# emdgroup/baybe

Measured on AMD Instinct MI355X. Metric: acquisition candidates scored/sec (1e6 discrete grid, n_train=512, qLogEI), higher is better.
Workload: dtype f64; 1 GPU; 1000000 x 20 discrete grid per GPU, n_train=512, Matern-5/2 ARD, qLogEI S=512, fixed-theta, top-8 to host; global_rows=1000000, parallelism=row-shard x1, collective=none

## Files before the change

baybe_amd/csrc/bbh_coop.h:

```cpp
#pragma once
#define BBH_CANDREG 1
#include "bbh_fused.h"

#define BBH_COOP_ROUNDS 8
#define BBH_COOP_KV_TILE (2 * 4 * 256)
#ifndef BBH_COOP_WAVES
#define BBH_COOP_WAVES 2
#endif
#ifndef BBH_COOP_PAIRS
#define BBH_COOP_PAIRS 4
#endif
#ifndef BBH_COOP_ABLATE_BARRIER
#define BBH_COOP_ABLATE_BARRIER 0
#endif
#ifndef BBH_COOP_ABLATE_MEM
#define BBH_COOP_ABLATE_MEM 0
#endif
#ifndef BBH_COOP_ABLATE_PRO
#define BBH_COOP_ABLATE_PRO 0
#endif
#ifndef BBH_COOP_ABLATE_LOADS
#define BBH_COOP_ABLATE_LOADS 0
#endif
#ifndef BBH_COOP_ABLATE_CHAIN
#define BBH_COOP_ABLATE_CHAIN 0
#endif
#ifndef BBH_COOP_ABLATE_KV
#define BBH_COOP_ABLATE_KV 0
#endif

typedef double d2 __attribute__((ext_vector_type(2)));
template <int IMM>
__device__ __forceinline__ void coop_gload2(d2& dst, const double* sbase, unsigned voff) {
  static_assert(IMM >= 0 && IMM + 16 <= 4096, "13-bit signed immediate offset");
  asm volatile("global_load_dwordx4 %0, %1, %2 offset:%3" : "=v"(dst) : "v"(voff), "s"(sbase), "n"(IMM));
}
template <int N>
__device__ __forceinline__ void coop_vmwait2(d2& slot) {
  asm volatile("s_waitcnt vmcnt(%1)" : "+v"(slot) : "n"(N));
}
template <int IMM>
__device__ __forceinline__ void coop_gload(double& dst, const double* sbase, unsigned voff) {
  static_assert(IMM >= 0 && IMM < 4096, "13-bit signed immediate offset");
  asm volatile("global_load_dwordx2 %0, %1, %2 offset:%3" : "=v"(dst) : "v"(voff), "s"(sbase), "n"(IMM));
}
template <int N>
__device__ __forceinline__ void coop_vmwait(double& slot) {
  asm volatile("s_waitcnt vmcnt(%1)" : "+v"(slot) : "n"(N));
}

struct CoopArgs {
  FusedArgs f;
  const double* rstream;
  int64_t frags;
  int g0;
  const double* na = nullptr;
};

__host__ __device__ constexpr int coop_frags_before(int G) { return 16 * (G * BBH_COOP_ROUNDS - (G * (G - 1)) / 2); }

template <int G, int KD, int KVF, bool PRODUCE, int NT, bool OPEN = false>
__device__ __forceinline__ void coop_group(const WaveCtx (&c)[NT], const double* rs, const double* tfn, const bbh_lds_double* kv_cur,
                                           bbh_lds_double* kv_mine_next, const bbh_lds_double* alpha_next, int tbn, int cw,
                                           d4 (&acc)[NT][BBH_COOP_ROUNDS], d2 (&ring)[BBH_COOP_PAIRS], double (&accm)[NT],
                                           const bbh_lds_double* na_next = (const bbh_lds_double*)nullptr) {
  constexpr bool SEED = (KVF & 8) != 0;
  constexpr int NP = BBH_COOP_PAIRS;
  constexpr int CNT = BBH_COOP_ROUNDS - G;
  constexpr int FULL = CNT - 1;
  constexpr int TOT = 16 * CNT;
  constexpr int REM = OPEN ? (1 << 20) : coop_frags_before(BBH_COOP_ROUNDS) - coop_frags_before(G + 1);
  constexpr int HOSTS = 12 * FULL;
  constexpr int STEPS = NT * BBH_KV_STEPS;
  const unsigned lane8 = (unsigned)c[0].l * 8u, lane16 = (unsigned)c[0].l * 16u;
  double tfv[KD];
  d4 dsa[NT], dsb[NT];
  KvState<BBH_KV_NU> P;
  double kv[NT][4], kvx[NT][4], kvn[NT][4], alv[4], nav[4];
  if constexpr (PRODUCE && SEED) {
#pragma unroll
    for (int r = 0; r < 4; r++) nav[r] = na_next[4 * r];
  }
  if constexpr (PRODUCE) {
    static_for<0, KD>([&](auto kc) __attribute__((always_inline)) {
      constexpr int k = decltype(kc)::value;
      coop_gload<(k % 8) * 512>(tfv[k], tfn + (k / 8) * 512, lane8);
    });
  }
#pragma unroll
  for (int t = 0; t < NT; t++)
#pragma unroll
    for (int r = 0; r < 4; r++) kv[t][r] = kv_cur[t * BBH_COOP_KV_TILE + r * 64];
  __builtin_amdgcn_sched_barrier(0);
  static_for<0, 4>([&](auto ic) __attribute__((always_inline)) {
    constexpr int i = decltype(ic)::value;
    if constexpr (i < 3) {
#pragma unroll
      for (int t = 0; t < NT; t++)
#pragma unroll
        for (int r = 0; r < 4; r++) kvx[t][r] = kv_cur[t * BBH_COOP_KV_TILE + (i + 1) * 256 + r * 64];
    } else if constexpr (PRODUCE) {
#pragma unroll
      for (int r = 0; r < 4; r++) alv[r] = alpha_next[4 * r];
    }
    static_for<0, 4>([&](auto rc) __attribute__((always_inline)) {
      constexpr int r = decltype(rc)::value;
      static_for<0, CNT>([&](auto sc) __attribute__((always_inline)) {
        constexpr int s = decltype(sc)::value;
        constexpr int f = (i * 4 + r) * CNT + s;
        constexpr int pr = f / 2;
        if constexpr (f % 2 == 0 && !BBH_COOP_ABLATE_LOADS) {
          constexpr int BEHIND = ((TOT + REM) / 2 - 1 - pr) < (NP - 1) ? ((TOT + REM) / 2 - 1 - pr) : (NP - 1);
          coop_vmwait2<BEHIND + ((PRODUCE && pr < NP) ? KD : 0)>(ring[pr % NP]);
        }
#if BBH_COOP_ABLATE_CHAIN
        static_for<0, NT>([&](auto tc_) __attribute__((always_inline)) {
          constexpr int t = decltype(tc_)::value;
          if constexpr (s == 0) {
            if (cw >= i) acc[t][f % 8] = mfma_f64(kv[t][r], ring[pr % NP][f % 2], acc[t][f % 8]);
          } else {
            acc[t][f % 8] = mfma_f64(kv[t][r], ring[pr % NP][f % 2], acc[t][f % 8]);
          }
        });
#else
        static_for<0, NT>([&](auto tc_) __attribute__((always_inline)) {
          constexpr int t = decltype(tc_)::value;
          if constexpr (s == 0) {
            if (cw >= i) acc[t][G] = mfma_f64(kv[t][r], ring[pr % NP][f % 2], acc[t][G]);
          } else {
            acc[t][G + s] = mfma_f64(kv[t][r], ring[pr % NP][f % 2], acc[t][G + s]);
          }
        });
#endif
        if constexpr (f % 2 == 1 && 2 * (pr + NP) < TOT + REM && !BBH_COOP_ABLATE_LOADS) {
          constexpr int np = pr + NP;
          coop_gload2<(np % 4) * 1024>(ring[pr % NP], BBH_COOP_ABLATE_MEM ? rs : rs + (np / 4) * 512, lane16);
        }
        if constexpr (PRODUCE && i >= 1 && s >= 1 && !BBH_COOP_ABLATE_KV) {
          constexpr int m = ((i - 1) * 4 + r) * FULL + (s - 1);
          static_for<(m * STEPS) / HOSTS, ((m + 1) * STEPS) / HOSTS>([&](auto st) __attribute__((always_inline)) {
            constexpr int tile = decltype(st)::value / BBH_KV_STEPS, micro = decltype(st)::value % BBH_KV_STEPS;
            kv_micro<KVF, BBH_KV_NU, micro>(P, c[tile], tbn, 0, dsa[tile], dsb[tile], kvn[tile]);
          });
        }
        __builtin_amdgcn_sched_barrier(0);
      });
      if constexpr (PRODUCE && i == 0 && r == 3) {
        coop_vmwait<NP>(tfv[KD - 1]);
        __builtin_amdgcn_sched_barrier(0);
        if constexpr (!BBH_COOP_ABLATE_KV) {
          static_for<0, NT>([&](auto tc_) __attribute__((always_inline)) {
            constexpr int t = decltype(tc_)::value;
            if constexpr (SEED) {
              const d4 seed = {nav[0] + c[t].nbn, nav[1] + c[t].nbn, nav[2] + c[t].nbn, nav[3] + c[t].nbn};
              kvp_dist_seeded<KD>(c[t], tfv, seed, dsa[t], dsb[t]);
            } else {
              kvp_dist<KD>(c[t], tfv, dsa[t], dsb[t]);
            }
          });
        }
      }
    });
    if constexpr (i < 3) {
#pragma unroll
      for (int t = 0; t < NT; t++)
#pragma unroll
        for (int r = 0; r < 4; r++) kv[t][r] = kvx[t][r];
    }
  });
  if constexpr (PRODUCE) {
#pragma unroll
    for (int t = 0; t < NT; t++)
#pragma unroll
      for (int r = 0; r < 4; r++) {
        if constexpr (BBH_COOP_ABLATE_KV) kvn[t][r] = tfv[r];
        kv_mine_next[t * BBH_COOP_KV_TILE + r * 64] = kvn[t][r];
        accm[t] = fma(kvn[t][r], alv[r], accm[t]);
      }
  }
}

template <int KD, int KVF, int NT, int GMIN = 0>
__global__ __launch_bounds__(256, (GMIN >= 6 ? 5 : GMIN >= 4 ? 4 : BBH_COOP_WAVES)) void bbh_coop_posterior_kernel(const CoopArgs ca) {
  const FusedArgs& a = ca.f;
  extern __shared__ __attribute__((aligned(16))) double s_mem[];
  constexpr bool SEED = (KVF & 8) != 0;
  static_assert(!SEED || (KVF & 6) == 0, "the seeded stream carries the Matern-5/2 constant");
  const int l = threadIdx.x & 63, w = __builtin_amdgcn_readfirstlane(threadIdx.x >> 6);
  const int cnd = l & 15, q = l >> 4;
  double* s_alpha = s_mem;
  double* s_na = s_alpha + 16 * a.nb;
  double* s_kv = s_na + (SEED ? 16 * a.nb : 0);
  double* s_red = s_kv + NT * BBH_COOP_KV_TILE;
  const int64_t tile0 = (int64_t)blockIdx.x * (16 * NT);

  WaveCtx c[NT];
  int tcs[NT];
  int xcol[KD];
  double xval[NT][KD], xscl[KD], xofs[KD];
  const double* xr[NT];
  double tfv0[KD];
  kvp_load<KD>(a.trainfrag + l, w, tfv0);
  double na0[4];
  if constexpr (SEED) {
#pragma unroll
    for (int r = 0; r < 4; r++) na0[r] = ca.na[16 * w + 4 * r + q];
  }
#pragma unroll
  for (int t = 0; t < NT; t++) {
    const int64_t row = (tile0 + 16 * t + cnd < a.N) ? tile0 + 16 * t + cnd : a.N - 1;
    xr[t] = a.X + row * a.ldx;
  }
  if (a.numcol_identity) {
#pragma unroll
    for (int k = 0; k < KD; k++) xcol[k] = (4 * k + q < a.dn) ? 4 * k + q : a.dn - 1;
  } else {
#pragma unroll
    for (int k = 0; k < KD; k++) xcol[k] = a.numcol[(4 * k + q < a.dn) ? 4 * k + q : a.dn - 1];
  }
#pragma unroll
  for (int k = 0; k < KD; k++) {
    const int dimc = (4 * k + q < a.dn) ? 4 * k + q : a.dn - 1;
#pragma unroll
    for (int t = 0; t < NT; t++) xval[t][k] = xr[t][xcol[k]];
    xscl[k] = a.scl[dimc];
    xofs[k] = a.ofs[dimc];
  }
  if (!(BBH_COOP_ABLATE_PRO & 1))
    for (int s = threadIdx.x; s < 16 * a.nb; s += 256) s_alpha[s] = a.meanB[(int64_t)s * 16];
  if constexpr (SEED)
    for (int s = threadIdx.x; s < 16 * a.nb; s += 256) s_na[s] = ca.na[s];
#pragma unroll
  for (int t = 0; t < NT; t++) {
    double nbsum = 0.0;
#pragma unroll
    for (int k = 0; k < KD; k++) {
      const int dim = 4 * k + q;
      double v = 0.0;
      if (dim < a.dn) {
        v = (BBH_COOP_ABLATE_PRO & 2) ? 0.01 * (double)(dim + cnd) : fma(xval[t][k], xscl[k], xofs[k]);
        if constexpr (SEED) v *= BBH_SQRT5;
        nbsum = fma(v, v, nbsum);
      }
      c[t].cf[k] = v;
    }
    nbsum += __shfl_xor(nbsum, 16, 64);
    nbsum += __shfl_xor(nbsum, 32, 64);
    if constexpr (!SEED) {
#pragma unroll
      for (int k = 0; k < KD; k++) {
        if (4 * k + q == a.dn) c[t].cf[k] = 1.0;
        if (4 * k + q == a.dn + 1) c[t].cf[k] = nbsum;
      }
    }
    c[t].nbn = nbsum;
    int tc = 0;
    if constexpr ((KVF & 1) != 0) {
      if (a.task_col >= 0) {
        tc = (int)xr[t][a.task_col];
        tc = tc < 0 ? 0 : (tc >= a.T ? a.T - 1 : tc);
      }
    }
    tcs[t] = tc;
    c[t].tf = a.trainfrag + l;
    c[t].candl = nullptr;
    c[t].mb = nullptr;
    c[t].tbl = a.tasktbl;
    c[t].taskext = a.taskext;
    c[t].kvc = nullptr;
    c[t].kvl = (bbh_lds_double*)nullptr;
    c[t].nl = 0;
    c[t].ncache = 0;
    c[t].al = (const bbh_lds_double*)nullptr;
    c[t].kd = KD;
    c[t].kind = a.kind;
    c[t].T = a.T;
    c[t].tc = tc;
    c[t].q = q;
    c[t].l = l;
    c[t].dn = a.dn;
  }

  bbh_lds_double* kvb = (bbh_lds_double*)(s_kv + l);
  const bbh_lds_double* alq = (const bbh_lds_double*)(s_alpha + q);
  const bbh_lds_double* naq = (const bbh_lds_double*)(s_na + q);
  const int g0 = ca.g0;
  double accm[NT];
  d4 acc[NT][BBH_COOP_ROUNDS];
#pragma unroll
  for (int t = 0; t < NT; t++) {
    accm[t] = 0.0;
#pragma unroll
    for (int s = 0; s < BBH_COOP_ROUNDS; s++) acc[t][s] = (d4){0.0, 0.0, 0.0, 0.0};
  }
  const double* rs = ca.rstream + (int64_t)w * ca.frags * 64;
  d2 ring[BBH_COOP_PAIRS];
  static_for<0, BBH_COOP_PAIRS>([&](auto ic) __attribute__((always_inline)) {
    constexpr int i = decltype(ic)::value;
    coop_gload2<(i % 4) * 1024>(ring[i], rs + (i / 4) * 512, (unsigned)l * 16u);
  });
  {
    double tfv[KD], kv0[NT][4];
    if constexpr (BBH_COOP_ABLATE_PRO & 4) {
      for (int t = 0; t < NT; t++)
        for (int r = 0; r < 4; r++) kv0[t][r] = 0.5 + 0.001 * (double)(l + r);
    } else {
#pragma unroll
      for (int k = 0; k < KD; k++) tfv[k] = tfv0[k];
#pragma unroll
      for (int t = 0; t < NT; t++) {
        d4 dsa, dsb;
        if constexpr (SEED) {
          const d4 seed = {na0[0] + c[t].nbn, na0[1] + c[t].nbn, na0[2] + c[t].nbn, na0[3] + c[t].nbn};
          kvp_dist_seeded<KD>(c[t], tfv, seed, dsa, dsb);
        } else {
          kvp_dist<KD>(c[t], tfv, dsa, dsb);
        }
        kv_all<KVF>(c[t], w, dsa, dsb, kv0[t]);
      }
    }
    __syncthreads();
#pragma unroll
    for (int t = 0; t < NT; t++)
#pragma unroll
      for (int r = 0; r < 4; r++) {
        kvb[t * BBH_COOP_KV_TILE + ((g0 & 1) * 4 + w) * 256 + r * 64] = kv0[t][r];
        accm[t] = fma(kv0[t][r], alq[16 * w + 4 * r], accm[t]);
      }
  }
  __syncthreads();

  static_for<GMIN, BBH_COOP_ROUNDS>([&](auto gc) __attribute__((always_inline)) {
    constexpr int G = decltype(gc)::value;
    if (G >= g0) {
      const int cw = (G & 1) ? 3 - w : w;
      const int tbn = 4 * (G + 1 - g0) + w;
      constexpr bool PRODUCE = G + 1 < BBH_COOP_ROUNDS;
      coop_group<G, KD, KVF, PRODUCE, NT>(c, rs, a.trainfrag + (int64_t)tbn * KD * 64, kvb + (G & 1) * 4 * 256,
                                          kvb + (((G + 1) & 1) * 4 + w) * 256, alq + 16 * tbn, tbn, cw, acc, ring, accm, naq + 16 * tbn);
      rs += (int64_t)16 * (BBH_COOP_ROUNDS - G) * 64;
#if !BBH_COOP_ABLATE_BARRIER
      if constexpr (PRODUCE) __syncthreads();
#endif
    }
  });

  if constexpr (BBH_COOP_ABLATE_PRO & 8) {
    double keep = 0.0;
#pragma unroll
    for (int t = 0; t < NT; t++) {
      keep += accm[t];
#pragma unroll
      for (int s = 0; s < BBH_COOP_ROUNDS; s++) keep += (acc[t][s][0] + acc[t][s][1]) + (acc[t][s][2] + acc[t][s][3]);
    }
    if (l == 0 && w == 0) a.var[tile0] = keep;
    return;
  }
#pragma unroll
  for (int t = 0; t < NT; t++) {
    double ss[4] = {0.0, 0.0, 0.0, 0.0};
#pragma unroll
    for (int s = 0; s < BBH_COOP_ROUNDS; s++)
#pragma unroll
      for (int r = 0; r < 4; r++) ss[r] = fma(acc[t][s][r], acc[t][s][r], ss[r]);
#pragma unroll
    for (int r = 0; r < 4; r++) {
      double v = ss[r];
      v += __shfl_xor(v, 1, 64);
      v += __shfl_xor(v, 2, 64);
      v += __shfl_xor(v, 4, 64);
      v += __shfl_xor(v, 8, 64);
      ss[r] = v;
    }
    double mp = accm[t];
    mp += __shfl_xor(mp, 16, 64);
    mp += __shfl_xor(mp, 32, 64);
    double* red_v = s_red + t * 128;
    double* red_m = red_v + 64;
    if (cnd == 0) {
#pragma unroll
      for (int r = 0; r < 4; r++) red_v[w * 16 + q + 4 * r] = ss[r];
    }
    if (q == 0) red_m[w * 16 + cnd] = mp;
  }
  __syncthreads();
  if (threadIdx.x < 16 * NT) {
    const int m = threadIdx.x & 15, t = threadIdx.x >> 4;
    const int64_t gi = tile0 + 16 * t + m;
    const double* red_v = s_red + t * 128;
    const double* red_m = red_v + 64;
    const double sv = (red_v[m] + red_v[16 + m]) + (red_v[32 + m] + red_v[48 + m]);
    const double sm = (red_m[m] + red_m[16 + m]) + (red_m[32 + m] + red_m[48 + m]);
    double pv = a.prior_scale, mc = a.mean_const;
    if constexpr ((KVF & 1) != 0) {
      int tcm = __shfl(tcs[0], m, 64);
      if constexpr (NT > 1) {
        const int tcm1 = __shfl(tcs[NT - 1], m, 64);
        tcm = t ? tcm1 : tcm;
      }
      pv = a.tasktbl[tcm * a.T + tcm];
      if (a.taskmean) mc = a.taskmean[tcm];
    }
    if (gi < a.N) {
      if (a.mean) a.mean[gi] = a.ybar + a.ysd * (mc + sm);
      if (a.var) a.var[gi] = a.ysd * a.ysd * (pv - sv);
    }
  }
}

bool bbh_coop_launch(int kd, int kind, bool has_tbl, dim3 grid, size_t lds, hipStream_t s, const CoopArgs& a, bool small_ok);
bool bbh_coop_launch_a(int kd, int kind, bool has_tbl, dim3 grid, size_t lds, hipStream_t s, const CoopArgs& a);
bool bbh_coop_launch_b(int kd, int kind, bool has_tbl, dim3 grid, size_t lds, hipStream_t s, const CoopArgs& a);
bool bbh_coop_launch_small(int kd, int kind, bool has_tbl, dim3 grid, size_t lds, hipStream_t s, const CoopArgs& a);
bool bbh_coop_seed_launch(int kds, bool has_tbl, dim3 grid, size_t lds, hipStream_t s, const CoopArgs& a, bool small_ok);
bool bbh_coop_seed_launch_small(int kds, bool has_tbl, dim3 grid, size_t lds, hipStream_t s, const CoopArgs& a);

#define BBH_COOP_DISPATCH_KD(KDV, NTV)                                                                                        \
  if (kd == KDV) {                                                                                                       \
    const bool m52 = kind == BBH_KERNEL_MATERN52, rbf = kind == BBH_KERNEL_RBF, plain = kind == BBH_KERNEL_MATERN32 && !has_tbl; \
    if (!m52 && !rbf && !plain) return false;                                                                            \
    if (grid.x == 0) return true;                                                                                        \
    if (rbf && has_tbl)                                                       \
      hipLaunchKernelGGL((bbh_coop_posterior_kernel<KDV, 3, NTV>), grid, dim3(256), lds, s, a);                               \
    else if (rbf)                                                                                                        \
      hipLaunchKernelGGL((bbh_coop_posterior_kernel<KDV, 2, NTV>), grid, dim3(256), lds, s, a);                               \
    else if (kind == BBH_KERNEL_MATERN32)                                                                                \
      hipLaunchKernelGGL((bbh_coop_posterior_kernel<KDV, 4, NTV>), grid, dim3(256), lds, s, a);                               \
    else if (has_tbl)                                                                                                    \
      hipLaunchKernelGGL((bbh_coop_posterior_kernel<KDV, 1, NTV>), grid, dim3(256), lds, s, a);                               \
    else                                                                                                                 \
      hipLaunchKernelGGL((bbh_coop_posterior_kernel<KDV, 0, NTV>), grid, dim3(256), lds, s, a);                               \
    return true;                                                                                                         \
  }
```

baybe_amd/csrc/bbh_fused.h:

```cpp
#pragma once
#include <math.h>
#include <string.h>

#include <type_traits>

#include "bbh_common.h"

#define BBH_MAX_PASS 64
#ifndef BBH_W32_REMAINDERS
#define BBH_W32_REMAINDERS 0
#endif

__device__ __forceinline__ double bbh_kfun_p(int kind, double r2) {
  if (kind == BBH_KERNEL_RBF) return exp(-0.5 * r2);
  const double r = sqrt(r2);
  if (kind == BBH_KERNEL_MATERN52) return (1.0 + BBH_SQRT5 * r + (5.0 / 3.0) * r2) * exp(-BBH_SQRT5 * r);
  if (kind == BBH_KERNEL_MATERN32) return (1.0 + BBH_SQRT3 * r) * exp(-BBH_SQRT3 * r);
  return exp(-r);
}

struct FusedArgs {
  const double* X;
  int64_t N, ldx;
  const double* trainfrag;
  const double* rfrag;
  const double* meanB;
  const double* scl;
  const double* ofs;
  const int* numcol;
  const double* tasktbl;
  const double* taskmean;
  const int* taskext;
  double* mean;
  double* var;
  double* cross;
  const int64_t* pass_off;
  const int* pass_w;
  int npass;
  int kind, dn, kd, nb, nb_ext, task_col, T, p, with_var;
  double ybar, ysd, mean_const, prior_scale;
  const double* qz;
  int qS;
  double q_best_f, q_sign;
  const uint8_t* q_alive;
  double* q_scores;
  double* kvcache;
  int* slab_flags;
  int nslab, nxcc;
  int ncache;
  int64_t nblk;
  int nl;
  int has_tbl;
  int mean_valu;
  int numcol_identity;
};

typedef __attribute__((address_space(3))) double bbh_lds_double;

struct WaveCtx {
  const double* tf;
  const double* candl;
  const double* mb;
  const double* tbl;
  const int* taskext;
  double* kvc;
  bbh_lds_double* kvl;
  int nl, ncache;
  const bbh_lds_double* al;
  int kd, kind, T, tc, q, l, dn;
  double nbn;
  double cf[16];
};

#ifndef BBH_CANDREG
#define BBH_CANDREG 0
#endif
#ifndef BBH_DIST_ASM
#define BBH_DIST_ASM 0
#endif
#ifndef BBH_MEAN_VALU_ONLY
#define BBH_MEAN_VALU_ONLY 0
#endif

template <bool HAS_TBL, int KIND>
__device__ __forceinline__ void compute_kv(const WaveCtx& c, int tb, double (&kv)[4]) {
  d4 da = {0.0, 0.0, 0.0, 0.0}, db = {0.0, 0.0, 0.0, 0.0};
  const double* tf = c.tf + (int64_t)tb * c.kd * 64;
  int k = 0;
  for (; k + 3 < c.kd; k += 4) {
    const double t0 = tf[k * 64], t1 = tf[(k + 1) * 64], t2 = tf[(k + 2) * 64], t3 = tf[(k + 3) * 64];
    const double c0 = c.candl[k * 64], c1 = c.candl[(k + 1) * 64], c2 = c.candl[(k + 2) * 64],
                 c3 = c.candl[(k + 3) * 64];
    da = mfma_f64(t0, c0, da);
    db = mfma_f64(t1, c1, db);
    da = mfma_f64(t2, c2, da);
    db = mfma_f64(t3, c3, db);
  }
  for (; k < c.kd; k++) da = mfma_f64(tf[k * 64], c.candl[k * 64], da);
#pragma unroll
  for (int r = 0; r < 4; r++) {
    const double r2 = fmax(da[r] + db[r], 0.0);
    double v;
    if (KIND == BBH_KERNEL_MATERN52) {
      const double rr = sqrt(r2);
      v = (1.0 + BBH_SQRT5 * rr + (5.0 / 3.0) * r2) * exp(-BBH_SQRT5 * rr);
    } else if (c.kind == BBH_KERNEL_MATERN12) {
      double d2 = r2;
      const bool nearp = r2 < 1e-2;
      if (__builtin_amdgcn_ballot_w64(nearp) != 0) {
        if (nearp) {
          const double* tfb = tf - c.l;
          const double* cb = c.candl - c.l;
          const int il = c.q + 4 * r, cl = c.l & 15;
          d2 = 0.0;
          for (int dim = 0; dim < c.dn; dim++) {
            const int o = (dim >> 2) * 64 + (dim & 3) * 16;
            const double df = cb[o + cl] + 0.5 * tfb[o + il];
            d2 = fma(df, df, d2);
          }
        }
      }
      v = (r2 > 1e7) ? 0.0 : exp(-sqrt(d2));
    } else {
      v = bbh_kfun_p(c.kind, r2);
    }
    if (HAS_TBL) v *= c.tbl[c.tc * c.T + c.taskext[16 * tb + 4 * r + c.q]];
    kv[r] = v;
  }
}

template <int W, int D, int TT, bool HAS_TBL, bool DO_MEAN, int KIND>
__device__ __forceinline__ void diag_steps(const WaveCtx& c, const double* rf, int j0, d4 (&acc)[W], double (&ring)[D],
                                           d4& accm) {
  if constexpr (TT < W) {
    constexpr int TOTAL = 2 * W * (W + 1);
    constexpr int BASE = 4 * (TT * W - (TT * (TT - 1)) / 2);
    constexpr int CNT = W - TT;
    double kv[4];
    double mbv[4];
    if (DO_MEAN) {
#pragma unroll
      for (int r = 0; r < 4; r++) mbv[r] = c.mb[(int64_t)(4 * (j0 + TT) + r) * 64];
    }
    compute_kv<HAS_TBL, KIND>(c, j0 + TT, kv);
    if (DO_MEAN) {
#pragma unroll
      for (int r = 0; r < 4; r++) accm = mfma_f64(kv[r], mbv[r], accm);
      __builtin_amdgcn_sched_barrier(0);
    }
#pragma unroll
    for (int r = 0; r < 4; r++)
#pragma unroll
      for (int jj = 0; jj < CNT; jj++) {
        const int i = BASE + r * CNT + jj;
        acc[TT + jj] = mfma_f64(kv[r], ring[i % D], acc[TT + jj]);
        if (i + D < TOTAL) ring[i % D] = rf[(i + D) * 64];
        if (i % D == D - 1) __builtin_amdgcn_sched_barrier(0);
      }
    diag_steps<W, D, TT + 1, HAS_TBL, DO_MEAN, KIND>(c, rf, j0, acc, ring, accm);
  }
}

template <int W, int D, bool HAS_TBL, bool DO_MEAN, int KIND>
__device__ __forceinline__ void pass_body(const WaveCtx& c, const double* rf, int j0, double (&ss)[4], d4& accm) {
  static_assert((4 * W) % D == 0 && (2 * W * (W + 1)) % D == 0, "ring depth must divide the stream");
  d4 acc[W];
#pragma unroll
  for (int jj = 0; jj < W; jj++) acc[jj] = (d4){0.0, 0.0, 0.0, 0.0};
  double ring[D];
#pragma unroll
  for (int i = 0; i < D; i++) ring[i] = rf[i * 64];
  for (int tb = 0; tb < j0; tb++) {
    double kv[4];
    double mbv[4];
    if (DO_MEAN) {
#pragma unroll
      for (int r = 0; r < 4; r++) mbv[r] = c.mb[(int64_t)(4 * tb + r) * 64];
    }
    compute_kv<HAS_TBL, KIND>(c, tb, kv);
    if (DO_MEAN) {
#pragma unroll
      for (int r = 0; r < 4; r++) accm = mfma_f64(kv[r], mbv[r], accm);
      __builtin_amdgcn_sched_barrier(0);
    }
#pragma unroll
    for (int i = 0; i < 4 * W; i++) {
      acc[i % W] = mfma_f64(kv[i / W], ring[i % D], acc[i % W]);
      ring[i % D] = rf[(i + D) * 64];
      if (i % D == D - 1) __builtin_amdgcn_sched_barrier(0);
    }
    rf += 4 * W * 64;
  }
  diag_steps<W, D, 0, HAS_TBL, DO_MEAN, KIND>(c, rf, j0, acc, ring, accm);
#pragma unroll
  for (int jj = 0; jj < W; jj++)
#pragma unroll
    for (int r = 0; r < 4; r++) ss[r] = fma(acc[jj][r], acc[jj][r], ss[r]);
}

template <int KD>
__device__ __forceinline__ void kvp_load(const double* tf_lane, int tb, double (&tfv)[KD]) {
  const double* tf = tf_lane + (int64_t)tb * KD * 64;
#pragma unroll
  for (int k = 0; k < KD; k++) tfv[k] = tf[k * 64];
}
template <int KD>
__device__ __forceinline__ void kvp_load(const WaveCtx& c, int tb, double (&tfv)[KD]) {
  kvp_load<KD>(c.tf, tb, tfv);
}

#if BBH_DIST_ASM
__device__ __forceinline__ void mfma_f64_v0(d4& acc, double a, double b) {
  asm volatile("v_mfma_f64_16x16x4_f64 %0, %1, %2, 0" : "=&v"(acc) : "v"(a), "v"(b));
}
__device__ __forceinline__ void mfma_f64_v(d4& acc, double a, double b) {
  asm volatile("v_mfma_f64_16x16x4_f64 %0, %1, %2, %0" : "+v"(acc) : "v"(a), "v"(b));
}
#endif

template <int KD>
__device__ __forceinline__ void kvp_dist(const WaveCtx& c, const double (&tfv)[KD], d4& da, d4& db) {
#if BBH_CANDREG && !BBH_DIST_ASM
  da = (d4){0.0, 0.0, 0.0, 0.0};
  db = (d4){0.0, 0.0, 0.0, 0.0};
#pragma unroll
  for (int k = 0; k < KD; k += 2) {
    da = mfma_f64(tfv[k], c.cf[k], da);
    if (k + 1 < KD) db = mfma_f64(tfv[k + 1], c.cf[k + 1], db);
  }
#elif BBH_CANDREG
  static_assert(KD >= 2, "two accumulator chains");
  mfma_f64_v0(da, tfv[0], c.cf[0]);
  mfma_f64_v0(db, tfv[1], c.cf[1]);
#pragma unroll
  for (int k = 2; k < KD; k += 2) {
    mfma_f64_v(da, tfv[k], c.cf[k]);
    if (k + 1 < KD) mfma_f64_v(db, tfv[k + 1], c.cf[k + 1]);
  }
#else
  da = (d4){0.0, 0.0, 0.0, 0.0};
  db = (d4){0.0, 0.0, 0.0, 0.0};
#pragma unroll
  for (int k = 0; k < KD; k += 2) {
    da = mfma_f64(tfv[k], c.candl[k * 64], da);
    if (k + 1 < KD) db = mfma_f64(tfv[k + 1], c.candl[(k + 1) * 64], db);
  }
#endif
}

template <int KD>
__device__ __forceinline__ void kvp_dist_seeded(const WaveCtx& c, const double (&tfv)[KD], const d4& seed, d4& da, d4& db) {
  static_assert(BBH_CANDREG && !BBH_DIST_ASM, "the seeded distance GEMM reads the candidate fragments from registers");
  da = seed;
  db = (d4){0.0, 0.0, 0.0, 0.0};
#pragma unroll
  for (int k = 0; k < KD; k += 2) {
    da = mfma_f64(tfv[k], c.cf[k], da);
    if (k + 1 < KD) db = mfma_f64(tfv[k + 1], c.cf[k + 1], db);
  }
}

#define BBH_KV_STEPS 18
#ifndef BBH_KV_SQRT_NR
#define BBH_KV_SQRT_NR 1
#endif
#ifndef BBH_KV_NU
#define BBH_KV_NU 4
#endif
template <int NU>
struct KvState {
  double t[NU], y[NU], g[NU], h[NU], kf[NU], q[NU], tv[NU];
  int ki[NU], te[NU];
};

#define BBH_KV_EACH for (int u = 0; u < NU; u++)
template <int I, int N, class F>
__device__ __forceinline__ void static_for(F&& f) {
  if constexpr (I < N) {
    f(std::integral_constant<int, I>{});
    static_for<I + 1, N>(f);
  }
}

template <int KVF, int NU, int step>
__device__ __forceinline__ void kv_micro(KvState<NU>& P, const WaveCtx& c, int tb, int r0, const d4& da, const d4& db,
                                         double (&out)[4]) {
  constexpr bool HAS_TBL = (KVF & 1) != 0, RBFK = (KVF & 2) != 0;
  constexpr bool PRESCALED = (KVF & 8) != 0;
  constexpr double RND = 6755399441055744.0;
  constexpr bool M32K = (KVF & 4) != 0;
  constexpr double KC1 = M32K ? 3.0 : 5.0, KC2 = M32K ? 0.0 : 1.0 / 3.0;
  constexpr double LOG2E = 1.4426950408889634074, LN2_HI = 6.93147180369123816490e-01,
                   LN2_LO = 1.90821492927058770002e-10;
  switch (step) {
    case 0:
#if BBH_DIST_ASM
      asm volatile("s_nop 15");
      asm volatile("s_nop 3");
#endif
#pragma unroll
      BBH_KV_EACH {
        const double r2 = da[r0 + u] + db[r0 + u];
        if (RBFK)
          P.g[u] = __builtin_fmin(__builtin_fmax(0.5 * r2, 0.0), 800.0);
        else
          P.t[u] = __builtin_fmax(PRESCALED ? r2 : KC1 * r2, 1e-300);
        if (HAS_TBL) P.te[u] = c.taskext[16 * tb + 4 * (r0 + u) + c.q];
      }
      break;
    case 1:
      if (RBFK) break;
#pragma unroll
      BBH_KV_EACH P.y[u] = __builtin_amdgcn_rsq(P.t[u]);
      break;
#if BBH_KV_SQRT_NR
    case 2:
      if (RBFK) break;
#pragma unroll
      BBH_KV_EACH P.g[u] = P.t[u] * P.y[u];
      break;
    case 3:
      if (RBFK) break;
#pragma unroll
      BBH_KV_EACH P.y[u] = fma(-P.g[u], P.y[u], 1.0);
      break;
    case 4:
      if (RBFK) break;
#pragma unroll
      BBH_KV_EACH P.h[u] = 0.5 * P.g[u];
      break;
    case 5: break;
    case 6:
      if (RBFK) break;
#pragma unroll
      BBH_KV_EACH P.g[u] = fma(P.h[u], P.y[u], P.g[u]);
      break;
#else
    case 2:
#pragma unroll
      BBH_KV_EACH P.g[u] = P.t[u] * P.y[u];
#pragma unroll
      BBH_KV_EACH P.h[u] = 0.5 * P.y[u];
      break;
    case 3:
#pragma unroll
      BBH_KV_EACH P.y[u] = fma(-P.h[u], P.g[u], 0.5);
      break;
    case 4:
#pragma unroll
      BBH_KV_EACH P.g[u] = fma(P.g[u], P.y[u], P.g[u]);
#pragma unroll
      BBH_KV_EACH P.h[u] = fma(P.h[u], P.y[u], P.h[u]);
      break;
    case 5:
#pragma unroll
      BBH_KV_EACH P.y[u] = fma(-P.g[u], P.g[u], P.t[u]);
      break;
    case 6:
#pragma unroll
      BBH_KV_EACH P.g[u] = __builtin_fmin(fma(P.y[u], P.h[u], P.g[u]), 800.0);
      break;
#endif
    case 7:
#pragma unroll
      BBH_KV_EACH P.y[u] = fma(P.g[u], -LOG2E, RND);
      if (!RBFK) {
#pragma unroll
        BBH_KV_EACH P.q[u] = M32K ? 1.0 : fma(P.g[u], KC2, 1.0);
#pragma unroll
        BBH_KV_EACH P.q[u] = fma(P.q[u], P.g[u], 1.0);
      }
      break;
    case 8:
#pragma unroll
      BBH_KV_EACH P.kf[u] = P.y[u] - RND;
#pragma unroll
      BBH_KV_EACH P.t[u] = fma(P.kf[u], -LN2_HI, -P.g[u]);
#pragma unroll
      BBH_KV_EACH P.t[u] = fma(P.kf[u], -LN2_LO, P.t[u]);
      break;
    case 9:
#pragma unroll
      BBH_KV_EACH {
        P.ki[u] = __double2loint(P.y[u]);
        if (HAS_TBL) P.tv[u] = c.tbl[c.tc * c.T + P.te[u]];
      }
      break;
    case 10:
#pragma unroll
      BBH_KV_EACH P.h[u] = fma(2.4994304884701822e-08, P.t[u], 2.763229327960932e-07);
      break;
#define BBH_KV_HORNER2(CA, CB)                      \
  _Pragma("unroll") BBH_KV_EACH P.h[u] = fma(P.h[u], P.t[u], CA); \
  _Pragma("unroll") BBH_KV_EACH P.h[u] = fma(P.h[u], P.t[u], CB);
    case 11: BBH_KV_HORNER2(2.7557622530873466e-06, 2.4801486521427063e-05) break;
    case 12: BBH_KV_HORNER2(0.00019841269432679235, 0.001388888895122399) break;
    case 13: BBH_KV_HORNER2(0.00833333333355927, 0.04166666666649277) break;
    case 14: BBH_KV_HORNER2(0.1666666666666617, 0.5000000000000018) break;
    case 15: BBH_KV_HORNER2(1.0, 1.0) break;
#undef BBH_KV_HORNER2
    case 16:
      if (!RBFK) {
#pragma unroll
        BBH_KV_EACH P.h[u] *= P.q[u];
      }
      break;
    default:
#pragma unroll
      BBH_KV_EACH {
        double v = __builtin_ldexp(P.h[u], P.ki[u]);
        if (HAS_TBL) v *= P.tv[u];
        out[r0 + u] = v;
      }
      break;
  }
}
#undef BBH_KV_EACH

template <int KVF>
__device__ __forceinline__ void kv_all(const WaveCtx& c, int tb, const d4& da, const d4& db, double (&out)[4]) {
  KvState<4> P;
  static_for<0, BBH_KV_STEPS>([&](auto st) __attribute__((always_inline)) {
    kv_micro<KVF, 4, decltype(st)::value>(P, c, tb, 0, da, db, out);
  });
}

#ifndef BBH_RING
#define BBH_RING 8
#endif
#define BBH_NEXT_NONE 0
#define BBH_NEXT_COMPUTE 1
#define BBH_NEXT_LOAD 2
template <int W, int CNT, int TT, int KD, int KVF, bool DO_MEAN, int NEXT, int BASE, int REM>
__device__ __forceinline__ void kblock_p(const WaveCtx& c, const double* rf, int tb, const double (&kv)[4],
                                         double (&kvn)[4], d4 (&acc)[W], d4& accm, double (&ring)[BBH_RING], bool store) {
  constexpr int D = BBH_RING;
  constexpr int TOT = 4 * CNT;
  double tfv[KD];
  d4 dsa, dsb;
  double mbv[4];
  KvState<BBH_KV_NU> P;
  if (NEXT == BBH_NEXT_COMPUTE) kvp_load<KD>(c, tb + 1, tfv);
  if (NEXT == BBH_NEXT_LOAD) {
    if (tb + 1 < c.nl) {
#pragma unroll
      for (int rr = 0; rr < 4; rr++) kvn[rr] = c.kvl[(tb + 1) * 256 + rr * 64];
    } else {
#pragma unroll
      for (int rr = 0; rr < 4; rr++) kvn[rr] = c.kvc[(int64_t)(tb + 1) * 256 + rr * 64];
    }
  }
  if (store && tb < c.ncache) {
#pragma unroll
    for (int rr = 0; rr < 4; rr++) {
      if (tb < c.nl)
        c.kvl[tb * 256 + rr * 64] = kv[rr];
      else
        c.kvc[(int64_t)tb * 256 + rr * 64] = kv[rr];
    }
  }
  __builtin_amdgcn_sched_barrier(0);
  static_for<0, 4>([&](auto rc) __attribute__((always_inline)) {
    constexpr int r = decltype(rc)::value;
    if (DO_MEAN && r == 3) {
      if (BBH_MEAN_VALU_ONLY || c.al) {
#pragma unroll
        for (int rr = 0; rr < 4; rr++) mbv[rr] = c.al[16 * tb + 4 * rr];
      } else {
#pragma unroll
        for (int rr = 0; rr < 4; rr++) mbv[rr] = c.mb[(int64_t)(4 * tb + rr) * 64];
      }
    }
    static_for<0, CNT>([&](auto jc) __attribute__((always_inline)) {
      constexpr int jj = decltype(jc)::value;
      constexpr int i = r * CNT + jj;
      acc[TT + jj] = mfma_f64(kv[r], ring[(BASE + i) % D], acc[TT + jj]);
      if (i + D < TOT + REM) ring[(BASE + i) % D] = rf[(i + D) * 64];
      if constexpr (NEXT == BBH_NEXT_COMPUTE && (r == 1 || r == 2)) {
        if constexpr (BBH_KV_NU == 4) {
          constexpr int m = (r - 1) * CNT + jj;
          static_for<(m * BBH_KV_STEPS) / (2 * CNT), ((m + 1) * BBH_KV_STEPS) / (2 * CNT)>(
              [&](auto st) __attribute__((always_inline)) {
                kv_micro<KVF, BBH_KV_NU, decltype(st)::value>(P, c, tb + 1, 0, dsa, dsb, kvn);
              });
        } else {
          static_for<(jj * BBH_KV_STEPS) / CNT, ((jj + 1) * BBH_KV_STEPS) / CNT>(
              [&](auto st) __attribute__((always_inline)) {
                kv_micro<KVF, BBH_KV_NU, decltype(st)::value>(P, c, tb + 1, 2 * (r - 1), dsa, dsb, kvn);
              });
        }
      }
      __builtin_amdgcn_sched_barrier(0);
    });
    if (NEXT == BBH_NEXT_COMPUTE && r == 0) kvp_dist<KD>(c, tfv, dsa, dsb);
    if (DO_MEAN && r == 3) {
      if (BBH_MEAN_VALU_ONLY || c.al) {
#pragma unroll
        for (int rr = 0; rr < 4; rr++) accm[0] = fma(kv[rr], mbv[rr], accm[0]);
      } else {
#pragma unroll
        for (int rr = 0; rr < 4; rr++) accm = mfma_f64(kv[rr], mbv[rr], accm);
      }
    }
    __builtin_amdgcn_sched_barrier(0);
  });
}

template <int W, int TT, int KD, int KVF, bool DO_MEAN>
__device__ __forceinline__ void diag_steps_p(const WaveCtx& c, const double* rf, int j0, double (&kv)[4], d4 (&acc)[W],
                                             d4& accm, double (&ring)[BBH_RING], bool store) {
  if constexpr (TT < W) {
    double kvn[4];
    constexpr int NEXT = (TT + 1 < W) ? BBH_NEXT_COMPUTE : BBH_NEXT_NONE;
    constexpr int BASE = (4 * (TT * W - (TT * (TT - 1)) / 2)) % BBH_RING;
    constexpr int REM = 2 * (W - TT) * (W - TT - 1);
    kblock_p<W, W - TT, TT, KD, KVF, DO_MEAN, NEXT, BASE, REM>(c, rf, j0 + TT, kv, kvn, acc, accm, ring, store);
    if (NEXT) {
#pragma unroll
      for (int r = 0; r < 4; r++) kv[r] = kvn[r];
    }
    diag_steps_p<W, TT + 1, KD, KVF, DO_MEAN>(c, rf + 4 * (W - TT) * 64, j0, kv, acc, accm, ring, store);
  }
}

template <int W, int KD, int KVF, bool DO_MEAN>
__device__ __forceinline__ void pass_body_p(const WaveCtx& c, const double* rf, int j0, double (&ss)[4], d4& accm,
                                            bool cache) {
  d4 acc[W];
#pragma unroll
  for (int jj = 0; jj < W; jj++) acc[jj] = (d4){0.0, 0.0, 0.0, 0.0};
  double kv[4], kvn[4], ring[BBH_RING];
#pragma unroll
  for (int i = 0; i < BBH_RING; i++) ring[i] = rf[i * 64];
  if (cache && j0 > 0) {
#pragma unroll
    for (int r = 0; r < 4; r++) {
      if (c.nl > 0)
        kv[r] = c.kvl[r * 64];
      else
        kv[r] = c.kvc[r * 64];
    }
  } else {
    double tfv[KD];
    d4 dsa, dsb;
    kvp_load<KD>(c, 0, tfv);
    kvp_dist<KD>(c, tfv, dsa, dsb);
    kv_all<KVF>(c, 0, dsa, dsb, kv);
  }
  const int nload = cache ? (j0 < c.ncache ? j0 : c.ncache) - 1 : 0;
  int tb = 0;
  for (; tb < nload; tb++) {
    kblock_p<W, W, 0, KD, KVF, DO_MEAN, BBH_NEXT_LOAD, 0, 1 << 20>(c, rf, tb, kv, kvn, acc, accm, ring, false);
#pragma unroll
    for (int r = 0; r < 4; r++) kv[r] = kvn[r];
    rf += 4 * W * 64;
  }
  for (; tb < j0; tb++) {
// ... 282 lines not shown
```

Measured before the change: 212.3 million candidates/s.

## Rework coop kernel prologue with scalar bases, bpermute shuffles, and splatted seed

Rewrites the cooperative posterior kernel prologue so loads use SGPR bases with unsigned byte offsets. The alpha and seed LDS fill is split into register loads issued early and stored after the setup work, and the LDS layout is reordered so alpha sits after the KV and reduction buffers. The seeded distance GEMM now takes a splatted norm vector as the second accumulator seed instead of per-element adds, and shuffles use ds_bpermute directly. The goal is to cut prologue latency, VALU work and register pressure, at the cost of added complexity and a residency heuristic table keyed on KD/GMIN.

Result: no change. 214.0 million candidates/s, median of 6 (+0.8%).

```diff
diff --git a/baybe_amd/csrc/bbh_coop.h b/baybe_amd/csrc/bbh_coop.h
--- a/baybe_amd/csrc/bbh_coop.h
+++ b/baybe_amd/csrc/bbh_coop.h
@@ -47,6 +47,27 @@
 template <int N>
 __device__ __forceinline__ void coop_vmwait(double& slot) {
   asm volatile("s_waitcnt vmcnt(%1)" : "+v"(slot) : "n"(N));
+}
+
+__device__ __forceinline__ int coop_sgpr(int v) {
+  asm volatile("" : "+s"(v));
+  return v;
+}
+
+template <class T>
+__device__ __forceinline__ T coop_ldg(const T* base, unsigned boff) {
+  typedef __attribute__((address_space(1))) const char gchar;
+  return *(const __attribute__((address_space(1))) T*)((gchar*)base + boff);
+}
+template <class T>
+__device__ __forceinline__ const T* coop_sbase(const T* p) {
+  asm volatile("" : "+s"(p));
+  return p;
+}
+template <int MASK>
+__device__ __forceinline__ double coop_shfl_xor(double v, unsigned l4) {
+  const int addr = (int)(l4 ^ (4u * MASK));
+  return __hiloint2double(__builtin_amdgcn_ds_bpermute(addr, __double2hiint(v)), __builtin_amdgcn_ds_bpermute(addr, __double2loint(v)));
 }
 
 struct CoopArgs {
@@ -59,7 +80,7 @@
 
 __host__ __device__ constexpr int coop_frags_before(int G) { return 16 * (G * BBH_COOP_ROUNDS - (G * (G - 1)) / 2); }
 
-template <int G, int KD, int KVF, bool PRODUCE, int NT, bool OPEN = false>
+template <int G, int KD, int KVF, bool PRODUCE, int NT, bool OPEN = false, bool SPLAT = true>
 __device__ __forceinline__ void coop_group(const WaveCtx (&c)[NT], const double* rs, const double* tfn, const bbh_lds_double* kv_cur,
                                            bbh_lds_double* kv_mine_next, const bbh_lds_double* alpha_next, int tbn, int cw,
                                            d4 (&acc)[NT][BBH_COOP_ROUNDS], d2 (&ring)[BBH_COOP_PAIRS], double (&accm)[NT],
@@ -76,7 +97,8 @@
   double tfv[KD];
   d4 dsa[NT], dsb[NT];
   KvState<BBH_KV_NU> P;
-  double kv[NT][4], kvx[NT][4], kvn[NT][4], alv[4], nav[4];
+  double kv[NT][4], kvx[NT][4], kvn[NT][4], alv[4];
+  d4 nav;
   if constexpr (PRODUCE && SEED) {
 #pragma unroll
     for (int r = 0; r < 4; r++) nav[r] = na_next[4 * r];
@@ -117,7 +139,7 @@
         static_for<0, NT>([&](auto tc_) __attribute__((always_inline)) {
           constexpr int t = decltype(tc_)::value;
           if constexpr (s == 0) {
-            if (cw >= i) acc[t][f % 8] = mfma_f64(kv[t][r], ring[pr % NP][f % 2], acc[t][f % 8]);
+            if (i == 0 || coop_sgpr(cw) >= i) acc[t][f % 8] = mfma_f64(kv[t][r], ring[pr % NP][f % 2], acc[t][f % 8]);
           } else {
             acc[t][f % 8] = mfma_f64(kv[t][r], ring[pr % NP][f % 2], acc[t][f % 8]);
           }
@@ -126,7 +148,7 @@
         static_for<0, NT>([&](auto tc_) __attribute__((always_inline)) {
           constexpr int t = decltype(tc_)::value;
           if constexpr (s == 0) {
-            if (cw >= i) acc[t][G] = mfma_f64(kv[t][r], ring[pr % NP][f % 2], acc[t][G]);
+            if (i == 0 || coop_sgpr(cw) >= i) acc[t][G] = mfma_f64(kv[t][r], ring[pr % NP][f % 2], acc[t][G]);
           } else {
             acc[t][G + s] = mfma_f64(kv[t][r], ring[pr % NP][f % 2], acc[t][G + s]);
           }
@@ -151,9 +173,11 @@
         if constexpr (!BBH_COOP_ABLATE_KV) {
           static_for<0, NT>([&](auto tc_) __attribute__((always_inline)) {
             constexpr int t = decltype(tc_)::value;
-            if constexpr (SEED) {
+            if constexpr (SEED && SPLAT) {
+              kvp_dist_seeded<KD>(c[t], tfv, nav, c[t].nbs, dsa[t], dsb[t]);
+            } else if constexpr (SEED) {
               const d4 seed = {nav[0] + c[t].nbn, nav[1] + c[t].nbn, nav[2] + c[t].nbn, nav[3] + c[t].nbn};
-              kvp_dist_seeded<KD>(c[t], tfv, seed, dsa[t], dsb[t]);
+              kvp_dist_seeded<KD>(c[t], tfv, seed, (d4){0.0, 0.0, 0.0, 0.0}, dsa[t], dsb[t]);
             } else {
               kvp_dist<KD>(c[t], tfv, dsa[t], dsb[t]);
             }
@@ -180,72 +204,98 @@
   }
 }
 
+__host__ __device__ constexpr bool coop_seed_resident(int KD, int KVF, int GMIN) {
+  const bool tbl = (KVF & 1) != 0;
+  if (GMIN >= 6) return false;
+  if (GMIN >= 4) return tbl ? (KD == 2 || KD == 4) : KD <= 5;
+  return KD == 12 || (tbl ? KD <= 3 : KD <= 7);
+}
+
 template <int KD, int KVF, int NT, int GMIN = 0>
 __global__ __launch_bounds__(256, (GMIN >= 6 ? 5 : GMIN >= 4 ? 4 : BBH_COOP_WAVES)) void bbh_coop_posterior_kernel(const CoopArgs ca) {
   const FusedArgs& a = ca.f;
   extern __shared__ __attribute__((aligned(16))) double s_mem[];
   constexpr bool SEED = (KVF & 8) != 0;
+  constexpr bool RESIDENT = !SEED || coop_seed_resident(KD, KVF, GMIN), SPLAT = SEED && RESIDENT;
   static_assert(!SEED || (KVF & 6) == 0, "the seeded stream carries the Matern-5/2 constant");
+  static_assert(BBH_COOP_KV_TILE + 128 >= 64 * BBH_COOP_ROUNDS, "the alpha base of the first round stays inside the LDS segment");
   const int l = threadIdx.x & 63, w = __builtin_amdgcn_readfirstlane(threadIdx.x >> 6);
   const int cnd = l & 15, q = l >> 4;
-  double* s_alpha = s_mem;
-  double* s_na = s_alpha + 16 * a.nb;
-  double* s_kv = s_na + (SEED ? 16 * a.nb : 0);
+  double* s_kv = s_mem;
   double* s_red = s_kv + NT * BBH_COOP_KV_TILE;
+  double* s_alpha = s_red + NT * 128;
   const int64_t tile0 = (int64_t)blockIdx.x * (16 * NT);
 
   WaveCtx c[NT];
   int tcs[NT];
-  int xcol[KD];
+  unsigned dim8[KD];
   double xval[NT][KD], xscl[KD], xofs[KD];
-  const double* xr[NT];
+  const double* xb[NT];
+  unsigned xrow[NT];
+  const unsigned l8 = (unsigned)l * 8u, l4 = (unsigned)l * 4u, q8 = (unsigned)q * 8u;
   double tfv0[KD];
-  kvp_load<KD>(a.trainfrag + l, w, tfv0);
-  double na0[4];
+  {
+    const double* tfw = coop_sbase(a.trainfrag + (int64_t)w * KD * 64);
+#pragma unroll
+    for (int k = 0; k < KD; k++) tfv0[k] = coop_ldg(tfw, l8 + 512u * k);
+  }
+  d4 na0;
   if constexpr (SEED) {
 #pragma unroll
-    for (int r = 0; r < 4; r++) na0[r] = ca.na[16 * w + 4 * r + q];
+    for (int r = 0; r < 4; r++) na0[r] = coop_ldg(ca.na + 16 * w + 4 * r, q8);
   }
 #pragma unroll
   for (int t = 0; t < NT; t++) {
-    const int64_t row = (tile0 + 16 * t + cnd < a.N) ? tile0 + 16 * t + cnd : a.N - 1;
-    xr[t] = a.X + row * a.ldx;
-  }
-  if (a.numcol_identity) {
-#pragma unroll
-    for (int k = 0; k < KD; k++) xcol[k] = (4 * k + q < a.dn) ? 4 * k + q : a.dn - 1;
-  } else {
-#pragma unroll
-    for (int k = 0; k < KD; k++) xcol[k] = a.numcol[(4 * k + q < a.dn) ? 4 * k + q : a.dn - 1];
-  }
+    const int64_t first = tile0 + 16 * t, left = a.N - 1 - first;
+    const int left_hi = coop_sgpr((int)(left >> 32)), left_lo = coop_sgpr((int)left);
+    const bool empty = left_hi < 0;
+    const int last = coop_sgpr(empty ? 0 : ((left_hi == 0 && (unsigned)left_lo < 16u) ? left_lo : 15));
+    xb[t] = a.X + (empty ? a.N - 1 : first) * a.ldx;
+    xrow[t] = (unsigned)(cnd < last ? cnd : last) * ((unsigned)a.ldx * 8u);
+  }
+  const unsigned dmax8 = (unsigned)(a.dn - 1) * 8u;
 #pragma unroll
   for (int k = 0; k < KD; k++) {
-    const int dimc = (4 * k + q < a.dn) ? 4 * k + q : a.dn - 1;
-#pragma unroll
-    for (int t = 0; t < NT; t++) xval[t][k] = xr[t][xcol[k]];
-    xscl[k] = a.scl[dimc];
-    xofs[k] = a.ofs[dimc];
-  }
-  if (!(BBH_COOP_ABLATE_PRO & 1))
-    for (int s = threadIdx.x; s < 16 * a.nb; s += 256) s_alpha[s] = a.meanB[(int64_t)s * 16];
-  if constexpr (SEED)
-    for (int s = threadIdx.x; s < 16 * a.nb; s += 256) s_na[s] = ca.na[s];
+    dim8[k] = (q8 + 32u * k < dmax8) ? q8 + 32u * k : dmax8;
+    xscl[k] = coop_ldg(a.scl, dim8[k]);
+    xofs[k] = coop_ldg(a.ofs, dim8[k]);
+  }
+  if (!a.numcol_identity) {
+#pragma unroll
+    for (int k = 0; k < KD; k++) dim8[k] = (unsigned)coop_ldg(a.numcol, dim8[k] >> 1) * 8u;
+  }
+#pragma unroll
+  for (int k = 0; k < KD; k++)
+#pragma unroll
+    for (int t = 0; t < NT; t++) xval[t][k] = coop_ldg(xb[t], xrow[t] + dim8[k]);
+  static_assert(16 * 4 * BBH_COOP_ROUNDS <= 2 * 256, "two values per thread fill alpha");
+  const int fill = 16 * a.nb - (int)threadIdx.x;
+  double fill_al[2], fill_na[2];
+  {
+    const double* src_al[2] = {coop_sbase(a.meanB), coop_sbase(a.meanB + 256 * 16)};
+    const double* src_na[2] = {SEED ? coop_sbase(ca.na) : nullptr, SEED ? coop_sbase(ca.na + 256) : nullptr};
+#pragma unroll
+    for (int j = 0; j < 2; j++) {
+      if (256 * j < fill) {
+        if (!(BBH_COOP_ABLATE_PRO & 1)) fill_al[j] = coop_ldg(src_al[j], threadIdx.x * 128u);
+        if constexpr (SEED) fill_na[j] = coop_ldg(src_na[j], threadIdx.x * 8u);
+      }
+    }
+  }
 #pragma unroll
   for (int t = 0; t < NT; t++) {
     double nbsum = 0.0;
 #pragma unroll
     for (int k = 0; k < KD; k++) {
       const int dim = 4 * k + q;
-      double v = 0.0;
-      if (dim < a.dn) {
-        v = (BBH_COOP_ABLATE_PRO & 2) ? 0.01 * (double)(dim + cnd) : fma(xval[t][k], xscl[k], xofs[k]);
-        if constexpr (SEED) v *= BBH_SQRT5;
-        nbsum = fma(v, v, nbsum);
-      }
+      double v = (BBH_COOP_ABLATE_PRO & 2) ? 0.01 * (double)(dim + cnd) : fma(xval[t][k], xscl[k], xofs[k]);
+      if constexpr (SEED) v *= BBH_SQRT5;
+      v = q8 + 32u * k <= dmax8 ? v : 0.0;
+      nbsum = fma(v, v, nbsum);
       c[t].cf[k] = v;
     }
-    nbsum += __shfl_xor(nbsum, 16, 64);
-    nbsum += __shfl_xor(nbsum, 32, 64);
+    nbsum += coop_shfl_xor<16>(nbsum, l4);
+    nbsum += coop_shfl_xor<32>(nbsum, l4);
     if constexpr (!SEED) {
 #pragma unroll
       for (int k = 0; k < KD; k++) {
@@ -254,10 +304,14 @@
       }
     }
     c[t].nbn = nbsum;
+    if constexpr (SPLAT) {
+      c[t].nbs = (d4){nbsum, nbsum, nbsum, nbsum};
+      asm volatile("" : "+v"(c[t].nbs));
+    }
     int tc = 0;
     if constexpr ((KVF & 1) != 0) {
       if (a.task_col >= 0) {
-        tc = (int)xr[t][a.task_col];
+        tc = (int)coop_ldg(xb[t], xrow[t] + (unsigned)a.task_col * 8u);
         tc = tc < 0 ? 0 : (tc >= a.T ? a.T - 1 : tc);
       }
     }
@@ -281,10 +335,22 @@
     c[t].dn = a.dn;
   }
 
+#pragma unroll
+  for (int j = 0; j < 2; j++) {
+    if (256 * j < fill) {
+      bbh_lds_double* dst = (bbh_lds_double*)s_alpha + threadIdx.x + 256 * j;
+      if (!(BBH_COOP_ABLATE_PRO & 1)) *dst = fill_al[j];
+      if constexpr (SEED) dst[16 * a.nb] = fill_na[j];
+    }
+  }
+
+  const int g0 = ca.g0;
   bbh_lds_double* kvb = (bbh_lds_double*)(s_kv + l);
-  const bbh_lds_double* alq = (const bbh_lds_double*)(s_alpha + q);
-  const bbh_lds_double* naq = (const bbh_lds_double*)(s_na + q);
-  const int g0 = ca.g0;
+  bbh_lds_double* kvw = kvb + w * 256;
+  const bbh_lds_double* alw = (const bbh_lds_double*)(s_alpha + q) + 16 * (w - 4 * g0);
+  const bbh_lds_double* naw = alw + 16 * a.nb;
+  if constexpr (RESIDENT) asm volatile("" : "+v"(kvw), "+v"(alw));
+  if constexpr (SPLAT) asm volatile("" : "+v"(naw));
   double accm[NT];
   d4 acc[NT][BBH_COOP_ROUNDS];
 #pragma unroll
@@ -310,9 +376,11 @@
 #pragma unroll
       for (int t = 0; t < NT; t++) {
         d4 dsa, dsb;
-        if constexpr (SEED) {
+        if constexpr (SPLAT) {
+          kvp_dist_seeded<KD>(c[t], tfv, na0, c[t].nbs, dsa, dsb);
+        } else if constexpr (SEED) {
           const d4 seed = {na0[0] + c[t].nbn, na0[1] + c[t].nbn, na0[2] + c[t].nbn, na0[3] + c[t].nbn};
-          kvp_dist_seeded<KD>(c[t], tfv, seed, dsa, dsb);
+          kvp_dist_seeded<KD>(c[t], tfv, seed, (d4){0.0, 0.0, 0.0, 0.0}, dsa, dsb);
         } else {
           kvp_dist<KD>(c[t], tfv, dsa, dsb);
         }
@@ -324,8 +392,8 @@
     for (int t = 0; t < NT; t++)
 #pragma unroll
       for (int r = 0; r < 4; r++) {
-        kvb[t * BBH_COOP_KV_TILE + ((g0 & 1) * 4 + w) * 256 + r * 64] = kv0[t][r];
-        accm[t] = fma(kv0[t][r], alq[16 * w + 4 * r], accm[t]);
+        kvw[t * BBH_COOP_KV_TILE + (g0 & 1) * 4 * 256 + r * 64] = kv0[t][r];
+        accm[t] = fma(kv0[t][r], alw[64 * g0 + 4 * r], accm[t]);
       }
   }
   __syncthreads();
@@ -336,8 +404,9 @@
       const int cw = (G & 1) ? 3 - w : w;
       const int tbn = 4 * (G + 1 - g0) + w;
       constexpr bool PRODUCE = G + 1 < BBH_COOP_ROUNDS;
-      coop_group<G, KD, KVF, PRODUCE, NT>(c, rs, a.trainfrag + (int64_t)tbn * KD * 64, kvb + (G & 1) * 4 * 256,
-                                          kvb + (((G + 1) & 1) * 4 + w) * 256, alq + 16 * tbn, tbn, cw, acc, ring, accm, naq + 16 * tbn);
+      coop_group<G, KD, KVF, PRODUCE, NT, false, SPLAT>(c, rs, a.trainfrag + (int64_t)tbn * KD * 64, kvb + (G & 1) * 4 * 256,
+                                                        kvw + ((G + 1) & 1) * 4 * 256, alw + 64 * (G + 1), tbn, cw, acc, ring, accm,
+                                                        naw + 64 * (G + 1));
       rs += (int64_t)16 * (BBH_COOP_ROUNDS - G) * 64;
 #if !BBH_COOP_ABLATE_BARRIER
       if constexpr (PRODUCE) __syncthreads();
@@ -366,15 +435,15 @@
 #pragma unroll
     for (int r = 0; r < 4; r++) {
       double v = ss[r];
-      v += __shfl_xor(v, 1, 64);
-      v += __shfl_xor(v, 2, 64);
-      v += __shfl_xor(v, 4, 64);
-      v += __shfl_xor(v, 8, 64);
+      v += coop_shfl_xor<1>(v, l4);
+      v += coop_shfl_xor<2>(v, l4);
+      v += coop_shfl_xor<4>(v, l4);
+      v += coop_shfl_xor<8>(v, l4);
       ss[r] = v;
     }
     double mp = accm[t];
-    mp += __shfl_xor(mp, 16, 64);
-    mp += __shfl_xor(mp, 32, 64);
+    mp += coop_shfl_xor<16>(mp, l4);
+    mp += coop_shfl_xor<32>(mp, l4);
     double* red_v = s_red + t * 128;
     double* red_m = red_v + 64;
     if (cnd == 0) {
diff --git a/baybe_amd/csrc/bbh_fused.h b/baybe_amd/csrc/bbh_fused.h
--- a/baybe_amd/csrc/bbh_fused.h
+++ b/baybe_amd/csrc/bbh_fused.h
@@ -69,6 +69,7 @@
   const bbh_lds_double* al;
   int kd, kind, T, tc, q, l, dn;
   double nbn;
+  d4 nbs;
   double cf[16];
 };
 
@@ -249,10 +250,11 @@
 }
 
 template <int KD>
-__device__ __forceinline__ void kvp_dist_seeded(const WaveCtx& c, const double (&tfv)[KD], const d4& seed, d4& da, d4& db) {
+__device__ __forceinline__ void kvp_dist_seeded(const WaveCtx& c, const double (&tfv)[KD], const d4& seeda, const d4& seedb, d4& da, d4& db) {
   static_assert(BBH_CANDREG && !BBH_DIST_ASM, "the seeded distance GEMM reads the candidate fragments from registers");
-  da = seed;
-  db = (d4){0.0, 0.0, 0.0, 0.0};
+  static_assert(KD >= 2, "two accumulator chains");
+  da = seeda;
+  db = seedb;
 #pragma unroll
   for (int k = 0; k < KD; k += 2) {
     da = mfma_f64(tfv[k], c.cf[k], da);
```
